# mttga/purejaxql

Measured on NVIDIA H100. Metric: MinAtar-Breakout env steps/sec @4096 envs x128 seeds, higher is better.
Workload: dtype f32

## Files before the change

purejaxql_b200/csrc/pqn_net.cu:

```cuda
#include <cuda_runtime.h>
#include <stdint.h>

#include "../../include/pqn_b200.h"
#include "api_common.h"
#include "tc_common.cuh"

namespace pqn {

constexpr int GT = 256;
constexpr int BK = 16;
constexpr float LN_EPS = 1e-6f;
constexpr int CONV_O = 16;
constexpr int CONV_PIX = 64;
constexpr int HID_CNN = 128;
constexpr int FLAT_CNN = CONV_PIX * CONV_O;

static int g_use_tc = 2;
static int g_conv_mma = 1;

__host__ __device__ static inline int64_t align4(int64_t x) { return (x + 3) & ~(int64_t)3; }

static int make_layout(const pqn_net_desc_t* d, pqn_net_layout_t* L) {
  int64_t off = 0;
  auto take = [&](int64_t n) { int64_t o = off; off += align4(n); return o; };
// ... 1050 lines not shown
      const uint32_t w0 = r00[(16 * i) * E::LD + ks], w1 = r00[(16 * i + 8) * E::LD + ks];
      a[i][0] = w0 & m_lo; a[i][1] = w1 & m_lo; a[i][2] = w0 & m_hi; a[i][3] = w1 & m_hi;
    }
    float2 bl[2], bh[2];
#pragma unroll
    for (int h = 0; h < 2; ++h) {
      bl[h] = wb_lo[(ks * 2 + h) * 32 + lane];
      bh[h] = wb_hi[(ks * 2 + h) * 32 + lane];
    }
#pragma unroll
    for (int h = 0; h < 2; ++h)
#pragma unroll
      for (int i = 0; i < 2; ++i) mma_tf32_16n8k8(z[i][h], a[i], __float_as_uint(bl[h].x), __float_as_uint(bl[h].y));
#pragma unroll
    for (int h = 0; h < 2; ++h)
#pragma unroll
      for (int i = 0; i < 2; ++i) mma_tf32_16n8k8(z[i][h], a[i], __float_as_uint(bh[h].x), __float_as_uint(bh[h].y));
  }
}

__device__ __forceinline__ void ln16_quad(const float (&z)[2][4], float& mean0, float& rstd0, float& mean1,
                                          float& rstd1) {
  float s0 = z[0][0] + z[0][1] + z[1][0] + z[1][1];
  float q0 = z[0][0] * z[0][0] + z[0][1] * z[0][1] + z[1][0] * z[1][0] + z[1][1] * z[1][1];
  float s1 = z[0][2] + z[0][3] + z[1][2] + z[1][3];
  float q1 = z[0][2] * z[0][2] + z[0][3] * z[0][3] + z[1][2] * z[1][2] + z[1][3] * z[1][3];
#pragma unroll
  for (int o = 1; o <= 2; o <<= 1) {
    s0 += __shfl_xor_sync(0xffffffffu, s0, o); q0 += __shfl_xor_sync(0xffffffffu, q0, o);
    s1 += __shfl_xor_sync(0xffffffffu, s1, o); q1 += __shfl_xor_sync(0xffffffffu, q1, o);
  }
  mean0 = s0 * (1.0f / CONV_O); mean1 = s1 * (1.0f / CONV_O);
  rstd0 = rsqrtf(fmaxf(q0 * (1.0f / CONV_O) - mean0 * mean0, 0.f) + LN_EPS);
  rstd1 = rsqrtf(fmaxf(q1 * (1.0f / CONV_O) - mean1 * mean1, 0.f) + LN_EPS);
}

constexpr int CONV_MMA_WARPS = 8;

template <int C, bool TRAIN, bool H16 = false>
__global__ void __launch_bounds__(CONV_MMA_WARPS * 32, 3)
    conv_fwd_mma_kernel(const uint32_t* __restrict__ obs, int64_t obs_rows_per_seed, const int32_t* __restrict__ gather,
                        const float* __restrict__ params, int64_t P, pqn_net_layout_t L, float* __restrict__ H1,
                        float* __restrict__ H1LO, float* __restrict__ XH1, float* __restrict__ RS1,
                        uint32_t* __restrict__ RB, float* __restrict__ bn_sums, int rows) {
  using Cfg = ConvCfg<C>;
  using M = ConvMma<C>;
  __shared__ float2 wb_hi[M::KS * 2 * 32], wb_lo[M::KS * 2 * 32];
  __shared__ float cb[CONV_O], sc[CONV_O], bi[CONV_O];
  __shared__ uint32_t so[CONV_MMA_WARPS][Cfg::SW];
  __shared__ uint32_t sxp[CONV_MMA_WARPS][CONV_PIX * ExpPatch<C>::LD];
  __shared__ float s_cnt[C];
  const int tid = threadIdx.x, warp = tid >> 5, lane = tid & 31;
  const int g = lane >> 2, t = lane & 3;
  const int seed = blockIdx.y;
  conv_mma_load_weights<C, true>(params + (int64_t)seed * P, L, wb_hi, wb_lo, cb, sc, bi);
  if (TRAIN && tid < C) s_cnt[tid] = 0.f;
  __syncthreads();
// ... 170 lines not shown
#pragma unroll
  for (int b = 0; b < 2 * Conv16<C>::KS; ++b) {
    const int o = 8 * b;
    uint32_t v = (o >> 5) < W ? w[(o >> 5) < W ? (o >> 5) : 0] : 0u;
    const int sh = o & 31;
    const uint32_t lo = sh >= 10 ? v >> (sh - 10) : v << (10 - sh);
    const uint32_t hi = sh + 4 <= 26 ? v << (26 - sh - 4) : v >> (sh + 4 - 26);
    out[b] = __byte_perm(lo, hi, 0x7610);
  }
}

template <int C>
__device__ __forceinline__ void store_patch16(const uint32_t* __restrict__ so, int pix, uint32_t* __restrict__ row) {
  using M = Conv16<C>;
  uint32_t w[M::ROW];
#pragma unroll
  for (int k = 0; k < M::ROW; ++k) w[k] = 0u;
  build_patch16<C>(so, pix, w);
#pragma unroll
  for (int q = 0; q < M::ROW / 4; ++q)
    *reinterpret_cast<uint4*>(row + 4 * q) = make_uint4(w[4 * q], w[4 * q + 1], w[4 * q + 2], w[4 * q + 3]);
}

template <int C>
__device__ __forceinline__ void conv16_block2(const uint32_t* __restrict__ xp, const uint4* __restrict__ wb,
                                              const float* __restrict__ cb, int mbp, int lane, float (&z)[2][2][4]) {
  using M = Conv16<C>;
  const int g = lane >> 2, t = lane & 3;
  const uint32_t mask = (1u << (10 + t)) | (1u << (26 + t));
#pragma unroll
  for (int i = 0; i < 2; ++i)
#pragma unroll
    for (int h = 0; h < 2; ++h) {
      z[i][h][0] = z[i][h][2] = cb[4 * t + 2 * h];
      z[i][h][1] = z[i][h][3] = cb[4 * t + 2 * h + 1];
    }
  const uint32_t* r00 = xp + (32 * mbp + g) * M::ROW;
#pragma unroll
  for (int s = 0; s < M::KS; ++s) {
    uint32_t a[2][4];
#pragma unroll
    for (int i = 0; i < 2; ++i) {
      const uint2 w0 = *reinterpret_cast<const uint2*>(r00 + (16 * i) * M::ROW + 2 * s);
      const uint2 w1 = *reinterpret_cast<const uint2*>(r00 + (16 * i + 8) * M::ROW + 2 * s);
      a[i][0] = w0.x & mask; a[i][1] = w1.x & mask; a[i][2] = w0.y & mask; a[i][3] = w1.y & mask;
    }
    uint4 b[2];
#pragma unroll
    for (int h = 0; h < 2; ++h) b[h] = wb[(s * 2 + h) * 32 + lane];
#pragma unroll
    for (int h = 0; h < 2; ++h)
#pragma unroll
      for (int i = 0; i < 2; ++i) mma_f16_16n8k16(z[i][h], a[i], b[h].z, b[h].w);
#pragma unroll
    for (int h = 0; h < 2; ++h)
#pragma unroll
      for (int i = 0; i < 2; ++i) mma_f16_16n8k16(z[i][h], a[i], b[h].x, b[h].y);
  }
}

__device__ __forceinline__ uint32_t cvt_f16x2_satfinite(float lo, float hi) {
  uint32_t r;
  asm("cvt.rn.satfinite.f16x2.f32 %0, %1, %2;" : "=r"(r) : "f"(hi), "f"(lo));
  return r;
}

constexpr int CONV16_WARPS = 4;
constexpr int CONV16_CTAS_PER_SM = 5;

template <int C, bool TRAIN, bool H16>
__global__ void __launch_bounds__(CONV16_WARPS * 32, CONV16_CTAS_PER_SM)
    conv_fwd_mma16_kernel(const uint32_t* __restrict__ obs, int64_t obs_rows_per_seed, const int32_t* __restrict__ gather,
                          const float* __restrict__ params, int64_t P, pqn_net_layout_t L, float* __restrict__ H1,
                          float* __restrict__ H1LO, float* __restrict__ XH1, float* __restrict__ RS1,
                          uint32_t* __restrict__ RB, float* __restrict__ bn_sums, int rows) {
  using Cfg = ConvCfg<C>;
  using M = Conv16<C>;
  __shared__ __align__(16) uint4 wb[M::KS * 2 * 32];
  __shared__ float cb[CONV_O], sc[CONV_O], bi[CONV_O];
  __shared__ uint32_t so[CONV16_WARPS][Cfg::SW];
  __shared__ __align__(16) uint32_t sxp[CONV16_WARPS][CONV_PIX * M::ROW];
  __shared__ float s_cnt[C];
  const int tid = threadIdx.x, warp = tid >> 5, lane = tid & 31;
  const int g = lane >> 2, t = lane & 3;
  const int seed = blockIdx.y;
  conv16_load_weights<C>(params + (int64_t)seed * P, L, wb, cb, sc, bi);
  if (TRAIN && tid < C) s_cnt[tid] = 0.f;
  __syncthreads();
  int cnt[C];
  uint32_t cmask[C];
#pragma unroll
  for (int c = 0; c < C; ++c) {
    cnt[c] = 0;
    cmask[c] = 0u;
    if (TRAIN) {
      for (int b = 0; b < 32; ++b) {
        const int f = lane * 32 + b;
        if (f < Cfg::OBS_BITS && f % C == c) cmask[c] |= 1u << b;
// ... 11 lines not shown
  auto fetch_obs = [&](int src) -> uint32_t {
    return __ldg(obs + ((int64_t)seed * obs_rows_per_seed + src) * Cfg::PW + (lane < Cfg::PW ? lane : 0));
  };
  const int row0 = blockIdx.x * CONV16_WARPS + warp;
  uint32_t pre = fetch_obs(fetch_index(row0));
  int src_next = fetch_index(row0 + row_stride);
  for (int row = row0; row < rows; row += row_stride) {
    __syncwarp();
    if (lane < Cfg::PW) my_so[lane] = pre;
    if (TRAIN && bn_sums != nullptr) {
#pragma unroll
      for (int c = 0; c < C; ++c) cnt[c] += __popc(pre & cmask[c]);
    }
    __syncwarp();
    pre = fetch_obs(src_next);
    src_next = fetch_index(row + 2 * row_stride);
    store_patch16<C>(my_so, lane, sxp[warp] + lane * M::ROW);
    store_patch16<C>(my_so, lane + 32, sxp[warp] + (lane + 32) * M::ROW);
    __syncwarp();
    const int64_t grow = (int64_t)seed * rows + row;
    float* __restrict__ hrow = H16 ? nullptr : H1 + grow * FLAT_CNN;
    __half* __restrict__ hrow16 = H16 ? reinterpret_cast<__half*>(H1) + grow * FLAT_CNN : nullptr;
    __half* __restrict__ lrow16 = H16 ? reinterpret_cast<__half*>(H1LO) + grow * FLAT_CNN : nullptr;
    float* __restrict__ xrow = (TRAIN && XH1) ? XH1 + grow * FLAT_CNN : nullptr;
    float* __restrict__ rrow = (TRAIN && RS1) ? RS1 + grow * CONV_PIX : nullptr;
    uint16_t* __restrict__ brow = (TRAIN && RB) ? reinterpret_cast<uint16_t*>(RB + grow * (FLAT_CNN / 32)) : nullptr;
    float keep_rs0 = 0.f, keep_rs1 = 0.f;
    uint32_t keep_rb = 0u;
#pragma unroll 1
    for (int mbp = 0; mbp < 2; ++mbp) {
      float z2[2][2][4];
      conv16_block2<C>(sxp[warp], wb, cb, mbp, lane, z2);
#pragma unroll
      for (int mi = 0; mi < 2; ++mi) {
        const int mb = 2 * mbp + mi;
        float (&z)[2][4] = z2[mi];
        float mean0, rstd0, mean1, rstd1;
        ln16_quad(z, mean0, rstd0, mean1, rstd1);
        const float nm0 = -mean0 * rstd0, nm1 = -mean1 * rstd1;
        uint32_t rb0 = 0u, rb1 = 0u;
        const int p0 = 16 * mb + g, p1 = p0 + 8, o4 = 4 * t;
        float x0[4], x1[4], v0[4], v1[4];
#pragma unroll
        for (int h = 0; h < 2; ++h) {
#pragma unroll
          for (int c = 0; c < 2; ++c) {
            const int o = o4 + 2 * h + c;
            x0[2 * h + c] = fmaf(z[h][c], rstd0, nm0);
            x1[2 * h + c] = fmaf(z[h][2 + c], rstd1, nm1);
            v0[2 * h + c] = fmaxf(fmaf(x0[2 * h + c], sc[o], bi[o]), 0.f);
            v1[2 * h + c] = fmaxf(fmaf(x1[2 * h + c], sc[o], bi[o]), 0.f);
          }
        }
        if (H16) {
          uint32_t hw0[2], hw1[2], lw0[2], lw1[2];
#pragma unroll
          for (int h = 0; h < 2; ++h) {
            hw0[h] = cvt_f16x2_satfinite(v0[2 * h], v0[2 * h + 1]);
            hw1[h] = cvt_f16x2_satfinite(v1[2 * h], v1[2 * h + 1]);
            const float2 f0 = __half22float2(*reinterpret_cast<const __half2*>(&hw0[h]));
            const float2 f1 = __half22float2(*reinterpret_cast<const __half2*>(&hw1[h]));
            const __half2 l0 = __floats2half2_rn((v0[2 * h] - f0.x) * tc::TC_LO_SCALE, (v0[2 * h + 1] - f0.y) * tc::TC_LO_SCALE);
            const __half2 l1 = __floats2half2_rn((v1[2 * h] - f1.x) * tc::TC_LO_SCALE, (v1[2 * h + 1] - f1.y) * tc::TC_LO_SCALE);
            lw0[h] = *reinterpret_cast<const uint32_t*>(&l0); lw1[h] = *reinterpret_cast<const uint32_t*>(&l1);
          }
          *reinterpret_cast<uint2*>(hrow16 + p0 * CONV_O + o4) = make_uint2(hw0[0], hw0[1]);
          *reinterpret_cast<uint2*>(lrow16 + p0 * CONV_O + o4) = make_uint2(lw0[0], lw0[1]);
          *reinterpret_cast<uint2*>(hrow16 + p1 * CONV_O + o4) = make_uint2(hw1[0], hw1[1]);
          *reinterpret_cast<uint2*>(lrow16 + p1 * CONV_O + o4) = make_uint2(lw1[0], lw1[1]);
        } else {
          *reinterpret_cast<float4*>(hrow + p0 * CONV_O + o4) = make_float4(v0[0], v0[1], v0[2], v0[3]);
          *reinterpret_cast<float4*>(hrow + p1 * CONV_O + o4) = make_float4(v1[0], v1[1], v1[2], v1[3]);
        }
        if (TRAIN) {
#pragma unroll
          for (int c = 0; c < 4; ++c) {
            rb0 |= (v0[c] > 0.f ? 1u : 0u) << (o4 + c);
            rb1 |= (v1[c] > 0.f ? 1u : 0u) << (o4 + c);
          }
        }
        if (xrow) {
          *reinterpret_cast<float4*>(xrow + p0 * CONV_O + o4) = make_float4(x0[0], x0[1], x0[2], x0[3]);
          *reinterpret_cast<float4*>(xrow + p1 * CONV_O + o4) = make_float4(x1[0], x1[1], x1[2], x1[3]);
          if (t == mb) { keep_rs0 = rstd0; keep_rs1 = rstd1; }
        }
        if (TRAIN && brow) {
          uint32_t rb = rb0 | (rb1 << 16);
          rb |= __shfl_xor_sync(0xffffffffu, rb, 1);
          rb |= __shfl_xor_sync(0xffffffffu, rb, 2);
          if (t == mb) keep_rb = rb;
        }
      }
    }
    if (TRAIN) {
      if (rrow) { rrow[16 * t + g] = keep_rs0; rrow[16 * t + g + 8] = keep_rs1; }
      if (brow) { brow[16 * t + g] = (uint16_t)keep_rb; brow[16 * t + g + 8] = (uint16_t)(keep_rb >> 16); }
    }
  }
  if (TRAIN && bn_sums != nullptr) {
#pragma unroll
    for (int c = 0; c < C; ++c) {
      int v = cnt[c];
#pragma unroll
      for (int o = 16; o > 0; o >>= 1) v += __shfl_xor_sync(0xffffffffu, v, o);
      if (lane == 0 && v) atomicAdd(&s_cnt[c], (float)v);
    }
    __syncthreads();
    if (tid < C && s_cnt[tid] != 0.f) {
      atomicAdd(bn_sums + (int64_t)seed * 2 * C + tid, s_cnt[tid]);
      atomicAdd(bn_sums + (int64_t)seed * 2 * C + C + tid, s_cnt[tid]);
    }
  }
}

constexpr int CDZ_LD = 16;
__device__ __forceinline__ int cswz(int p, int col) { return col ^ (((p >> 1) & 1) << 3); }

__device__ __forceinline__ void cp_async16(void* smem_dst, const void* gsrc) {
  asm volatile("cp.async.cg.shared.global [%0], [%1], 16;" ::"r"((uint32_t)__cvta_generic_to_shared(smem_dst)), "l"(gsrc)
               : "memory");
// ... 211 lines not shown
    if (warp == w && g == 0) {
#pragma unroll
      for (int col = 0; col < 4; ++col) {
        const int o = 8 * (col >> 1) + 2 * t + (col & 1);
        s_red[o] = (w == 0 ? 0.f : s_red[o]) + a_dsc[col];
        s_red[CONV_O + o] = (w == 0 ? 0.f : s_red[CONV_O + o]) + a_dbi[col];
        s_red[2 * CONV_O + o] = (w == 0 ? 0.f : s_red[2 * CONV_O + o]) + a_dcb[col];
      }
    }
    __syncthreads();
  }
  float* __restrict__ o = part + ((int64_t)seed * gridDim.x + blockIdx.x) * (M::TAPS * CONV_O + 3 * CONV_O);
  for (int i = tid; i < M::TAPS * CONV_O; i += blockDim.x) o[i] = s_w[i] * (1.0f / 255.0f);
  if (tid < 3 * CONV_O) o[M::TAPS * CONV_O + tid] = s_red[tid];
}

template <int C>
struct ConvBwd16 {
  static constexpr int MT = ConvMma<C>::MT;
  static constexpr int NG = 4 * MT;
  static constexpr int NGP = (NG % 8 == 4) ? NG : NG + 4;
  static constexpr int DY = 0;
  static constexpr int XH = DY + FLAT_CNN;
  static constexpr int RS = XH + FLAT_CNN;
  static constexpr int DZT = RS + CONV_PIX;
  static constexpr int PW = DZT + 2 * CONV_O * 32;
  static constexpr int WARP_FLOATS = (PW + 32 * NGP + 3) / 4 * 4;
  static constexpr int WARPS = (C == 4) ? 8 : 6;
  static constexpr int BYTES = (WARPS * WARP_FLOATS + 4 * CONV_O) * 4;
};

__device__ __forceinline__ int cswz16(int p, int col) {
  return ((p ^ ((p >> 2) & 1)) << 4) + (col ^ (((p >> 1) & 1) << 3));
}
__device__ __forceinline__ int dzt_word(int ch, int ks, int pos) {
  const int c7 = ch & 7;
  return (ch << 5) + ((ks ^ ((c7 + (c7 >> 2)) & 3)) << 3) + pos;
}

template <int C>
__global__ void __launch_bounds__(ConvBwd16<C>::WARPS * 32, 2)
    conv_bwd_mma16_kernel(const uint32_t* __restrict__ obs, int64_t obs_rows_per_seed, const int32_t* __restrict__ gather,
                          const float* __restrict__ params, int64_t P, pqn_net_layout_t L, const float* __restrict__ DY1,
                          const float* __restrict__ XH1, const float* __restrict__ RS1, float* __restrict__ part,
                          int rows, float gs) {
  using Cfg = ConvCfg<C>;
  using M = ConvMma<C>;
  using SM = ConvBwd16<C>;
  constexpr int PWD = PatchCfg<C>::WORDS;
  extern __shared__ __align__(16) float smem_bwd[];
  const int tid = threadIdx.x, warp = tid >> 5, lane = tid & 31;
  const int g = lane >> 2, t = lane & 3;
  const int seed = blockIdx.y;
  float* my = smem_bwd + warp * SM::WARP_FLOATS;
  float* my_dy = my + SM::DY;
  float* my_xh = my + SM::XH;
  float* my_rs = my + SM::RS;
  uint32_t* my_dzt = reinterpret_cast<uint32_t*>(my + SM::DZT);
  uint32_t* my_so = reinterpret_cast<uint32_t*>(my + SM::DZT);
  uint32_t* my_pw = reinterpret_cast<uint32_t*>(my + SM::PW);
  float* sc = smem_bwd + SM::WARPS * SM::WARP_FLOATS;
  float* s_red = sc + CONV_O;
  float* s_w = smem_bwd;
  static_assert(Cfg::SW <= 2 * CONV_O * 32, "obs staging aliases the dz planes");
  static_assert(M::MT * 16 * CONV_O <= SM::WARP_FLOATS * SM::WARPS, "dW reduction buffer aliases the warp slices");
  static_assert(Cfg::PW <= 32, "one packed observation word per lane");
  if (tid < CONV_O) sc[tid] = __ldg(params + (int64_t)seed * P + L.ln0_scale + tid);
  if (tid < 3 * CONV_O) s_red[tid] = 0.f;
  __syncthreads();
  float a_dsc[4] = {0.f, 0.f, 0.f, 0.f}, a_dbi[4] = {0.f, 0.f, 0.f, 0.f}, a_dcb[4] = {0.f, 0.f, 0.f, 0.f};
  float wrun[M::MT][2][4];
#pragma unroll
  for (int mt = 0; mt < M::MT; ++mt)
#pragma unroll
    for (int h = 0; h < 2; ++h)
#pragma unroll
      for (int j = 0; j < 4; ++j) wrun[mt][h][j] = 0.f;
  const uint32_t amask = (1u << (10 + (g & 3))) | (1u << (26 + (g & 3)));
  const int pos_g = g < 4 ? 2 * g : 2 * (g - 4) + 1;

  const int row_stride = gridDim.x * SM::WARPS;
  auto fetch_index = [&](int r) -> int {
    const int rc = r < rows ? r : rows - 1;
    return gather ? __ldg(gather + (int64_t)seed * rows + rc) : rc;
  };
  auto fetch_obs = [&](int src) -> uint32_t {
    return __ldg(obs + ((int64_t)seed * obs_rows_per_seed + src) * Cfg::PW + (lane < Cfg::PW ? lane : 0));
  };
  auto fetch_rows = [&](int r) {
    if (r < rows) {
      const int64_t gr = (int64_t)seed * rows + r;
      const float* dsrc = DY1 + gr * FLAT_CNN;
      const float* xsrc = XH1 + gr * FLAT_CNN;
#pragma unroll
      for (int i = 0; i < FLAT_CNN / 4 / 32; ++i) {
        const int q = i * 32 + lane, prow = q >> 2;
        const int dst = cswz16(prow, (q & 3) * 4);
        cp_async16(my_dy + dst, dsrc + q * 4);
        cp_async16(my_xh + dst, xsrc + q * 4);
      }
      if (lane < CONV_PIX / 4) cp_async16(my_rs + lane * 4, RS1 + gr * CONV_PIX + lane * 4);
    }
    cp_async_commit();
  };
  int row = blockIdx.x * SM::WARPS + warp;
  uint32_t pre = fetch_obs(fetch_index(row));
  int src_next = fetch_index(row + row_stride);
  fetch_rows(row);
  for (; row < rows; row += row_stride) {
    __syncwarp();
    if (lane < Cfg::PW) my_so[lane] = pre;
    if (lane == 0) my_so[Cfg::PW] = 0u;
    __syncwarp();
    pre = fetch_obs(src_next);
    src_next = fetch_index(row + 2 * row_stride);
    {
      uint32_t w0[PWD], w1[PWD];
      patch_bits<C>(my_so, 2 * lane, w0);
      patch_bits<C>(my_so, 2 * lane + 1, w1);
      uint32_t pw[SM::NGP];
#pragma unroll
      for (int k = 0; k < SM::NGP; ++k) pw[k] = 0u;
#pragma unroll
      for (int q = 0; q < SM::NG; ++q) {
        const int ql = q & 3, slot = (q & ~3) + (ql == 1 ? 2 : (ql == 2 ? 1 : ql));
        const int bit = 4 * q, wi = bit >> 5, sh = bit & 31;
        if (wi < PWD) {
          const uint32_t v0 = w0[wi < PWD ? wi : 0], v1 = w1[wi < PWD ? wi : 0];
          const uint32_t lo = sh >= 10 ? v0 >> (sh >= 10 ? sh - 10 : 0) : v0 << (sh < 10 ? 10 - sh : 0);
          const uint32_t hi = sh <= 26 ? v1 << (sh <= 26 ? 26 - sh : 0) : v1 >> (sh > 26 ? sh - 26 : 0);
          pw[slot] = __byte_perm(lo, hi, 0x7610);
        }
      }
      uint32_t* dstw = my_pw + lane * SM::NGP;
#pragma unroll
      for (int k = 0; k < SM::NGP / 4; ++k)
        *reinterpret_cast<uint4*>(dstw + 4 * k) = make_uint4(pw[4 * k], pw[4 * k + 1], pw[4 * k + 2], pw[4 * k + 3]);
    }
    cp_async_wait_all();
    __syncwarp();
#pragma unroll 1
    for (int mb = 0; mb < 4; ++mb) {
      const int p0 = 16 * mb + 2 * g, p1 = p0 + 1;
      float z[2][4];
      float2 dyv[2][2];
#pragma unroll
      for (int h = 0; h < 2; ++h) {
        dyv[h][0] = *reinterpret_cast<const float2*>(my_dy + cswz16(p0, 8 * h + 2 * t));
        dyv[h][1] = *reinterpret_cast<const float2*>(my_dy + cswz16(p1, 8 * h + 2 * t));
        const float2 a0 = *reinterpret_cast<const float2*>(my_xh + cswz16(p0, 8 * h + 2 * t));
        const float2 a1 = *reinterpret_cast<const float2*>(my_xh + cswz16(p1, 8 * h + 2 * t));
        z[h][0] = a0.x; z[h][1] = a0.y; z[h][2] = a1.x; z[h][3] = a1.y;
      }
      const float rstd0 = my_rs[p0] * gs, rstd1 = my_rs[p1] * gs;
      float dxh[2][4];
      float m1a = 0.f, m2a = 0.f, m1b = 0.f, m2b = 0.f;
#pragma unroll
      for (int h = 0; h < 2; ++h) {
        const int o = 8 * h + 2 * t;
        const float dy4[4] = {dyv[h][0].x, dyv[h][0].y, dyv[h][1].x, dyv[h][1].y};
#pragma unroll
        for (int j = 0; j < 4; ++j) {
          const int col = 2 * h + (j & 1);
          a_dsc[col] = fmaf(dy4[j], z[h][j], a_dsc[col]);
          a_dbi[col] += dy4[j];
          dxh[h][j] = dy4[j] * sc[o + (j & 1)];
          if (j < 2) { m1a += dxh[h][j]; m2a = fmaf(dxh[h][j], z[h][j], m2a); }
          else { m1b += dxh[h][j]; m2b = fmaf(dxh[h][j], z[h][j], m2b); }
        }
      }
#pragma unroll
      for (int o = 1; o <= 2; o <<= 1) {
        m1a += __shfl_xor_sync(0xffffffffu, m1a, o); m2a += __shfl_xor_sync(0xffffffffu, m2a, o);
        m1b += __shfl_xor_sync(0xffffffffu, m1b, o); m2b += __shfl_xor_sync(0xffffffffu, m2b, o);
      }
      m1a *= (1.0f / CONV_O); m2a *= (1.0f / CONV_O); m1b *= (1.0f / CONV_O); m2b *= (1.0f / CONV_O);
#pragma unroll
      for (int h = 0; h < 2; ++h) {
        float dzv[4];
#pragma unroll
        for (int j = 0; j < 4; ++j) {
          const float rstd = j < 2 ? rstd0 : rstd1, m1 = j < 2 ? m1a : m1b, m2 = j < 2 ? m2a : m2b;
          dzv[j] = rstd * (dxh[h][j] - m1 - z[h][j] * m2);
          a_dcb[2 * h + (j & 1)] += dzv[j];
        }
#pragma unroll
        for (int c = 0; c < 2; ++c) {
          const float v0 = dzv[c], v1 = dzv[2 + c];
          const uint32_t hw = cvt_f16x2_satfinite(v0, v1);
          const float2 hf = __half22float2(*reinterpret_cast<const __half2*>(&hw));
          const __half2 lw = __floats2half2_rn(v0 - hf.x, v1 - hf.y);
          const int wd = dzt_word(8 * h + 2 * t + c, mb, pos_g);
          my_dzt[wd] = hw;
          my_dzt[CONV_O * 32 + wd] = *reinterpret_cast<const uint32_t*>(&lw);
        }
      }
    }
    __syncwarp();
    fetch_rows(row + row_stride);
    float wacc[M::MT][2][4];
#pragma unroll
    for (int mt = 0; mt < M::MT; ++mt)
#pragma unroll
      for (int h = 0; h < 2; ++h)
#pragma unroll
        for (int j = 0; j < 4; ++j) wacc[mt][h][j] = 0.f;
#pragma unroll 1
    for (int ks = 0; ks < 4; ++ks) {
      uint2 bhi[2], blo[2];
#pragma unroll
      for (int h = 0; h < 2; ++h) {
        const int wd = dzt_word(8 * h + g, ks, 2 * t);
        bhi[h] = *reinterpret_cast<const uint2*>(my_dzt + wd);
        blo[h] = *reinterpret_cast<const uint2*>(my_dzt + CONV_O * 32 + wd);
      }
      const uint32_t* pa = my_pw + (8 * ks + t) * SM::NGP + 2 * (g >> 2);
      const uint32_t* pb = pa + 4 * SM::NGP;
#pragma unroll
      for (int mt = 0; mt < M::MT; ++mt) {
        const uint2 wa = *reinterpret_cast<const uint2*>(pa + 4 * mt), wb = *reinterpret_cast<const uint2*>(pb + 4 * mt);
        uint32_t a[4];
        a[0] = wa.x & amask; a[1] = wa.y & amask; a[2] = wb.x & amask; a[3] = wb.y & amask;
// ... 289 lines not shown
}


template <int C>
static int launch_conv_bwd_mma(dim3 grid, cudaStream_t st, const uint32_t* obs, int64_t orps, const int32_t* gather,
                               const float* params, int64_t P, const pqn_net_layout_t& L, const float* dy1,
                               const float* xh1, const float* rs1, float* grads, float* part, int rows) {
  auto kfn = conv_bwd_mma_kernel<C>;
  if (cudaFuncSetAttribute(kfn, cudaFuncAttributeMaxDynamicSharedMemorySize, ConvBwdSmem<C>::BYTES) != cudaSuccess)
    return check_launch("conv_bwd_mma(cudaFuncSetAttribute)");
  kfn<<<grid, ConvBwdSmem<C>::WARPS * 32, ConvBwdSmem<C>::BYTES, st>>>(obs, orps, gather, params, P, L, dy1, xh1, rs1,
                                                                       part, rows);
  const int n = 9 * C * CONV_O + 3 * CONV_O;
  if (final_slices((int)grid.x) == 32)
    conv_bwd_final_kernel<32><<<dim3(cdiv(n, 8), grid.y), 256, 0, st>>>(part, (int)grid.x, 9 * C * CONV_O, grads, P, L);
  else
    conv_bwd_final_kernel<8><<<dim3(cdiv(n, 32), grid.y), 256, 0, st>>>(part, (int)grid.x, 9 * C * CONV_O, grads, P, L);
  return 0;
}

template <int C>
static int launch_conv_bwd_mma16(dim3 grid, cudaStream_t st, const uint32_t* obs, int64_t orps, const int32_t* gather,
                                 const float* params, int64_t P, const pqn_net_layout_t& L, const float* dy1,
                                 const float* xh1, const float* rs1, float* grads, float* part, int rows, float gs) {
  auto kfn = conv_bwd_mma16_kernel<C>;
  if (cudaFuncSetAttribute(kfn, cudaFuncAttributeMaxDynamicSharedMemorySize, ConvBwd16<C>::BYTES) != cudaSuccess)
    return check_launch("conv_bwd_mma16(cudaFuncSetAttribute)");
  kfn<<<grid, ConvBwd16<C>::WARPS * 32, ConvBwd16<C>::BYTES, st>>>(obs, orps, gather, params, P, L, dy1, xh1, rs1, part,
                                                                   rows, gs);
  const int n = 9 * C * CONV_O + 3 * CONV_O;
  if (final_slices((int)grid.x) == 32)
    conv_bwd_final_kernel<32><<<dim3(cdiv(n, 8), grid.y), 256, 0, st>>>(part, (int)grid.x, 9 * C * CONV_O, grads, P, L);
  else
    conv_bwd_final_kernel<8><<<dim3(cdiv(n, 32), grid.y), 256, 0, st>>>(part, (int)grid.x, 9 * C * CONV_O, grads, P, L);
  return 0;
}

static size_t row_bwd_smem(int N, int A, bool head) {
  return (size_t)(24 * N + (head ? A * N + 8 * A + 16 + 8 * A * N : 0)) * sizeof(float);
}
static int64_t row_bwd_part_floats(int N, int A) { return 3 * (int64_t)N + (int64_t)A * N + A + 2; }

template <int N, bool HEAD, typename... Args>
static int launch_row_bwd(dim3 grid, int A, cudaStream_t st, Args... args) {
  const size_t sm = row_bwd_smem(N, A, HEAD);
  if (sm > 48 * 1024 &&
      cudaFuncSetAttribute(row_bwd_kernel<N, HEAD>, cudaFuncAttributeMaxDynamicSharedMemorySize, (int)sm) != cudaSuccess)
    return check_launch("row_bwd(cudaFuncSetAttribute)");
  LaunchScope _ls(K_ROW_BWD, st);
  row_bwd_kernel<N, HEAD><<<grid, 256, sm, st>>>(args...);
  return 0;
}
// ... 41 lines not shown
  const int maxc = (rows + CONV_MMA_WARPS - 1) / CONV_MMA_WARPS;
  int best = 1;
  double best_eff = 0.0;
  const int lim = (6 * resident + S - 1) / S;
  for (int per_seed = 1; per_seed <= lim && per_seed <= maxc; ++per_seed) {
    const int total = per_seed * S;
    const int waves = (total + resident - 1) / resident;
    if (waves > 6) break;
    const double eff = (double)total / ((double)waves * resident);
    if (eff > best_eff + 0.01 || (eff > best_eff - 0.01 && waves <= 4)) { best_eff = eff > best_eff ? eff : best_eff; best = per_seed; }
  }
  return (unsigned)best;
}

template <bool TRAIN>
static int launch_conv_fwd(int C, dim3 grid, cudaStream_t st, const uint32_t* obs, int64_t orps, const int32_t* gather,
                           const float* params, int64_t P, const pqn_net_layout_t& L, float* h1, float* h1lo, float* bn,
                           int rows, float* xh1 = nullptr, float* rs1 = nullptr, uint32_t* rb = nullptr,
                           bool h16 = false) {
  if (g_conv_mma == 1) {
    const dim3 mg(conv_mma_ctas((int)grid.y, rows, CONV16_CTAS_PER_SM), grid.y);
    LaunchScope _ls(TRAIN ? K_CONV_FWD : K_CONV_FWD_INFER, st);
#define PQN_CONV16(CC)                                                                                              \
  if (h16) conv_fwd_mma16_kernel<CC, TRAIN, true><<<mg, CONV16_WARPS * 32, 0, st>>>(obs, orps, gather, params, P, L, h1, h1lo, xh1, rs1, rb, bn, rows); \
  else conv_fwd_mma16_kernel<CC, TRAIN, false><<<mg, CONV16_WARPS * 32, 0, st>>>(obs, orps, gather, params, P, L, h1, h1lo, xh1, rs1, rb, bn, rows)
    switch (C) {
      case 4: PQN_CONV16(4); break;
      case 6: PQN_CONV16(6); break;
      case 7: PQN_CONV16(7); break;
      case 10: PQN_CONV16(10); break;
      default: return -1;
    }
#undef PQN_CONV16
    return 0;
  }
  if (g_conv_mma == 3) {
    const dim3 mg(conv_mma_ctas((int)grid.y, rows, 3), grid.y);
    LaunchScope _ls(TRAIN ? K_CONV_FWD : K_CONV_FWD_INFER, st);
    switch (C) {
      case 4: conv_fwd_mma_kernel<4, TRAIN><<<mg, CONV_MMA_WARPS * 32, 0, st>>>(obs, orps, gather, params, P, L, h1, h1lo, xh1, rs1, rb, bn, rows); break;
      case 6: conv_fwd_mma_kernel<6, TRAIN><<<mg, CONV_MMA_WARPS * 32, 0, st>>>(obs, orps, gather, params, P, L, h1, h1lo, xh1, rs1, rb, bn, rows); break;
      case 7: conv_fwd_mma_kernel<7, TRAIN><<<mg, CONV_MMA_WARPS * 32, 0, st>>>(obs, orps, gather, params, P, L, h1, h1lo, xh1, rs1, rb, bn, rows); break;
      case 10: conv_fwd_mma_kernel<10, TRAIN><<<mg, CONV_MMA_WARPS * 32, 0, st>>>(obs, orps, gather, params, P, L, h1, h1lo, xh1, rs1, rb, bn, rows); break;
      default: return -1;
    }
    return 0;
  }
  switch (C) {
// ... 628 lines not shown
  const int64_t P = L.total;
  Workspace w;
  carve(d, S, rows, (char*)workspace, &w);
  const int A = d->num_actions;
  const int R = (int)rows;
  if (cudaMemsetAsync(grads, 0, (size_t)S * P * sizeof(float), st) != cudaSuccess)
    return check_launch("pqn_qnet_loss_grad(memset)");
  if (modular_net(d)) {
    nrm::NormWs nw;
    nrm::carve_norm(d, S, rows, (char*)workspace, &nw);
    return nrm::norm_loss_grad(d, L, params, batch_stats, obs, gather, obs_rows_per_seed, action, target, tr_rows_per_seed,
                              grads, loss_sum, qsa_sum, bn_sums, S, R, nw, st);
  }

  if (d->kind == PQN_NET_MINATAR_CNN) {
    const uint32_t* ob = (const uint32_t*)obs;
    const bool use_tc = g_use_tc && A <= PQN_TC_MAX_A;
    const bool f16 = use_tc && g_use_tc == 2;
    const Planes16 pl = planes16(w, S, rows);
    const bool conv16 = f16 && g_conv_mma == 1;
    const float gscale = f16 ? grad_scale(rows) : 1.0f;
    launch_conv_fwd<true>(d->in_c, dim3(cdiv(rows, 4), S), st, ob, obs_rows_per_seed, gather, params, P, L,
                          conv16 ? (float*)pl.h1_hi : w.h1, conv16 ? (float*)pl.h1_lo : nullptr, bn_sums, R,
                          g_conv_mma ? w.cxhat : nullptr, g_conv_mma ? w.crstd : nullptr,
                          (g_conv_mma == 1 || g_conv_mma == 3) ? w.relu_bits : nullptr, conv16);
    if (f16) {
      if (!conv16) launch_split16_h1(w.h1, pl, (int64_t)S * rows * FLAT_CNN, st);
      launch_split16_w1(params, P, L.d0_w, pl, S, st);
      if ((rc = tc16_dense_fwd(tc::EPI_LN_TRAIN, params, P, L, w, pl, A, nullptr, S, R, st))) return rc;
    } else if (use_tc) {
      launch_split_w1(params, P, L.d0_w, w.w1_lo, S, st);
      if ((rc = tc_dense_fwd(tc::EPI_LN_TRAIN, params, P, L, w, A, nullptr, S, R, st))) return rc;
    } else {
      if ((rc = launch_dense<1>(128, dim3(cdiv(rows, 128), S), st, w.h1, rows * FLAT_CNN, FLAT_CNN, params, P, L.d0_w, L.d0_b,
                      L.ln1_scale, L.ln1_bias, 0, 0, A, w.h2, w.xhat2, w.rstd2, nullptr, R, FLAT_CNN))) return rc;
    }
    const dim3 rbg(conv_mma_ctas(S, R, 4), S);
    if ((rc = run_row_bwd(128, true, rbg, A, st, w.h2, w.xhat2, w.rstd2, nullptr, w.dz2, (use_tc && !f16) ? w.dz2_lo : nullptr,
                          f16 ? pl.dz_hi : nullptr, f16 ? pl.dz_lo : nullptr, gscale, params, grads, P, L.ln1_scale,
                          L.ln1_bias, L.d0_b, L.head_w, L.head_b, gather, action, target, tr_rows_per_seed, loss_sum,
                          qsa_sum, w.rb_part, R))) return rc;
    if (f16) {
      if ((rc = tc16_wgrad(grads, P, L, pl, S, R, gscale, w.wg_part, st))) return rc;
      if ((rc = tc16_dgrad(w, pl, S, R, g_conv_mma == 1 || g_conv_mma == 3, gscale, st))) return rc;
    } else if (use_tc) {
      if ((rc = tc_wgrad(grads, P, L, w, S, R, st))) return rc;
      if ((rc = tc_dgrad(params, P, L, w, S, R, g_conv_mma == 1 || g_conv_mma == 3, st))) return rc;
    } else {
      const int splits = wgrad_splits(FLAT_CNN / 128, S, R);
      run_wgrad_ffma(w.h1, rows * FLAT_CNN, FLAT_CNN, w.dz2, rows * HID_CNN, HID_CNN, grads, P, L.d0_w, R, FLAT_CNN, S, splits, w.wg_part, st);
      launch_dgrad(w.dz2, rows * HID_CNN, HID_CNN, params, P, L.d0_w, w.h1, w.h1, rows * FLAT_CNN, R, FLAT_CNN, 0, S, st);
    }
    dim3 cg(conv_bwd_ctas(S, R), S);
    if (g_conv_mma) {
      const dim3 mg(conv_mma_ctas(S, R, 2), S);
      LaunchScope _ls(K_CONV_BWD, st);
      const float gs16 = grad_scale((int)rows) * (1.0f / 16.0f);
      if (g_conv_mma == 1) {
        switch (d->in_c) {
          case 4: rc = launch_conv_bwd_mma16<4>(mg, st, ob, obs_rows_per_seed, gather, params, P, L, w.h1, w.cxhat, w.crstd, grads, w.cb_part, R, gs16); break;
          case 6: rc = launch_conv_bwd_mma16<6>(mg, st, ob, obs_rows_per_seed, gather, params, P, L, w.h1, w.cxhat, w.crstd, grads, w.cb_part, R, gs16); break;
          case 7: rc = launch_conv_bwd_mma16<7>(mg, st, ob, obs_rows_per_seed, gather, params, P, L, w.h1, w.cxhat, w.crstd, grads, w.cb_part, R, gs16); break;
          case 10: rc = launch_conv_bwd_mma16<10>(mg, st, ob, obs_rows_per_seed, gather, params, P, L, w.h1, w.cxhat, w.crstd, grads, w.cb_part, R, gs16); break;
        }
      } else
      switch (d->in_c) {
        case 4: rc = launch_conv_bwd_mma<4>(mg, st, ob, obs_rows_per_seed, gather, params, P, L, w.h1, w.cxhat, w.crstd, grads, w.cb_part, R); break;
        case 6: rc = launch_conv_bwd_mma<6>(mg, st, ob, obs_rows_per_seed, gather, params, P, L, w.h1, w.cxhat, w.crstd, grads, w.cb_part, R); break;
        case 7: rc = launch_conv_bwd_mma<7>(mg, st, ob, obs_rows_per_seed, gather, params, P, L, w.h1, w.cxhat, w.crstd, grads, w.cb_part, R); break;
        case 10: rc = launch_conv_bwd_mma<10>(mg, st, ob, obs_rows_per_seed, gather, params, P, L, w.h1, w.cxhat, w.crstd, grads, w.cb_part, R); break;
      }
      if (rc) return rc;
    } else
    switch (d->in_c) {
      case 4: { LaunchScope _ls(K_CONV_BWD, st); conv_bwd_kernel<4><<<cg, 256, 0, st>>>(ob, obs_rows_per_seed, gather, params, P, L, w.h1, grads, R); } break;
      case 6: { LaunchScope _ls(K_CONV_BWD, st); conv_bwd_kernel<6><<<cg, 256, 0, st>>>(ob, obs_rows_per_seed, gather, params, P, L, w.h1, grads, R); } break;
      case 7: { LaunchScope _ls(K_CONV_BWD, st); conv_bwd_kernel<7><<<cg, 256, 0, st>>>(ob, obs_rows_per_seed, gather, params, P, L, w.h1, grads, R); } break;
      case 10: { LaunchScope _ls(K_CONV_BWD, st); conv_bwd_kernel<10><<<cg, 256, 0, st>>>(ob, obs_rows_per_seed, gather, params, P, L, w.h1, grads, R); } break;
    }
  } else {
    const int D = d->in_c, H = d->hidden;
    const int BM = (H == 128) ? 128 : 64;
    const bool bits = d->kind == PQN_NET_MLP_BITS, bits_tc = bits && g_use_tc == 2;
    const uint32_t* ob = (const uint32_t*)obs;
    bits::BitsWs bw = {};
    if (bits) bits::carve_bits(d, S, rows, (char*)workspace + carve(d, S, rows, nullptr, nullptr), &bw);
// ... 66 lines not shown
```

Before: 33.51 million.

## Recompute conv LayerNorm xhat and rstd in backward instead of storing them

```diff
diff --git a/purejaxql_b200/csrc/pqn_net.cu b/purejaxql_b200/csrc/pqn_net.cu
--- a/purejaxql_b200/csrc/pqn_net.cu
+++ b/purejaxql_b200/csrc/pqn_net.cu
@@ -1096,17 +1096,17 @@
 __device__ __forceinline__ void ln16_quad(const float (&z)[2][4], float& mean0, float& rstd0, float& mean1,
                                           float& rstd1) {
   float s0 = z[0][0] + z[0][1] + z[1][0] + z[1][1];
-  float q0 = z[0][0] * z[0][0] + z[0][1] * z[0][1] + z[1][0] * z[1][0] + z[1][1] * z[1][1];
+  float q0 = fmaf(z[1][1], z[1][1], fmaf(z[1][0], z[1][0], fmaf(z[0][0], z[0][0], __fmul_rn(z[0][1], z[0][1]))));
   float s1 = z[0][2] + z[0][3] + z[1][2] + z[1][3];
-  float q1 = z[0][2] * z[0][2] + z[0][3] * z[0][3] + z[1][2] * z[1][2] + z[1][3] * z[1][3];
+  float q1 = fmaf(z[1][3], z[1][3], fmaf(z[1][2], z[1][2], fmaf(z[0][2], z[0][2], __fmul_rn(z[0][3], z[0][3]))));
 #pragma unroll
   for (int o = 1; o <= 2; o <<= 1) {
     s0 += __shfl_xor_sync(0xffffffffu, s0, o); q0 += __shfl_xor_sync(0xffffffffu, q0, o);
     s1 += __shfl_xor_sync(0xffffffffu, s1, o); q1 += __shfl_xor_sync(0xffffffffu, q1, o);
   }
-  mean0 = s0 * (1.0f / CONV_O); mean1 = s1 * (1.0f / CONV_O);
-  rstd0 = rsqrtf(fmaxf(q0 * (1.0f / CONV_O) - mean0 * mean0, 0.f) + LN_EPS);
-  rstd1 = rsqrtf(fmaxf(q1 * (1.0f / CONV_O) - mean1 * mean1, 0.f) + LN_EPS);
+  mean0 = __fmul_rn(s0, 1.0f / CONV_O); mean1 = __fmul_rn(s1, 1.0f / CONV_O);
+  rstd0 = rsqrtf(fmaxf(fmaf(q0, 1.0f / CONV_O, -__fmul_rn(mean0, mean0)), 0.f) + LN_EPS);
+  rstd1 = rsqrtf(fmaxf(fmaf(q1, 1.0f / CONV_O, -__fmul_rn(mean1, mean1)), 0.f) + LN_EPS);
 }
 
 constexpr int CONV_MMA_WARPS = 8;
@@ -1323,25 +1323,25 @@
     *reinterpret_cast<uint4*>(row + 4 * q) = make_uint4(w[4 * q], w[4 * q + 1], w[4 * q + 2], w[4 * q + 3]);
 }
 
-template <int C>
-__device__ __forceinline__ void conv16_block2(const uint32_t* __restrict__ xp, const uint4* __restrict__ wb,
-                                              const float* __restrict__ cb, int mbp, int lane, float (&z)[2][2][4]) {
+template <int C, int NB>
+__device__ __forceinline__ void conv16_blocks(const uint32_t* __restrict__ xp, const uint4* __restrict__ wb,
+                                              const float* __restrict__ cb, int mb0, int lane, float (&z)[NB][2][4]) {
   using M = Conv16<C>;
   const int g = lane >> 2, t = lane & 3;
   const uint32_t mask = (1u << (10 + t)) | (1u << (26 + t));
 #pragma unroll
-  for (int i = 0; i < 2; ++i)
+  for (int i = 0; i < NB; ++i)
 #pragma unroll
     for (int h = 0; h < 2; ++h) {
       z[i][h][0] = z[i][h][2] = cb[4 * t + 2 * h];
       z[i][h][1] = z[i][h][3] = cb[4 * t + 2 * h + 1];
     }
-  const uint32_t* r00 = xp + (32 * mbp + g) * M::ROW;
+  const uint32_t* r00 = xp + (16 * mb0 + g) * M::ROW;
 #pragma unroll
   for (int s = 0; s < M::KS; ++s) {
-    uint32_t a[2][4];
-#pragma unroll
-    for (int i = 0; i < 2; ++i) {
+    uint32_t a[NB][4];
+#pragma unroll
+    for (int i = 0; i < NB; ++i) {
       const uint2 w0 = *reinterpret_cast<const uint2*>(r00 + (16 * i) * M::ROW + 2 * s);
       const uint2 w1 = *reinterpret_cast<const uint2*>(r00 + (16 * i + 8) * M::ROW + 2 * s);
       a[i][0] = w0.x & mask; a[i][1] = w1.x & mask; a[i][2] = w0.y & mask; a[i][3] = w1.y & mask;
@@ -1352,12 +1352,26 @@
 #pragma unroll
     for (int h = 0; h < 2; ++h)
 #pragma unroll
-      for (int i = 0; i < 2; ++i) mma_f16_16n8k16(z[i][h], a[i], b[h].z, b[h].w);
+      for (int i = 0; i < NB; ++i) mma_f16_16n8k16(z[i][h], a[i], b[h].z, b[h].w);
 #pragma unroll
     for (int h = 0; h < 2; ++h)
 #pragma unroll
-      for (int i = 0; i < 2; ++i) mma_f16_16n8k16(z[i][h], a[i], b[h].x, b[h].y);
-  }
+      for (int i = 0; i < NB; ++i) mma_f16_16n8k16(z[i][h], a[i], b[h].x, b[h].y);
+  }
+}
+
+__device__ __forceinline__ void conv16_xhat(const float (&z)[2][4], float (&x0)[4], float (&x1)[4], float& rstd0,
+                                            float& rstd1) {
+  float mean0, mean1;
+  ln16_quad(z, mean0, rstd0, mean1, rstd1);
+  const float nm0 = -__fmul_rn(mean0, rstd0), nm1 = -__fmul_rn(mean1, rstd1);
+#pragma unroll
+  for (int h = 0; h < 2; ++h)
+#pragma unroll
+    for (int c = 0; c < 2; ++c) {
+      x0[2 * h + c] = fmaf(z[h][c], rstd0, nm0);
+      x1[2 * h + c] = fmaf(z[h][2 + c], rstd1, nm1);
+    }
 }
 
 __device__ __forceinline__ uint32_t cvt_f16x2_satfinite(float lo, float hi) {
@@ -1373,8 +1387,7 @@
 __global__ void __launch_bounds__(CONV16_WARPS * 32, CONV16_CTAS_PER_SM)
     conv_fwd_mma16_kernel(const uint32_t* __restrict__ obs, int64_t obs_rows_per_seed, const int32_t* __restrict__ gather,
                           const float* __restrict__ params, int64_t P, pqn_net_layout_t L, float* __restrict__ H1,
-                          float* __restrict__ H1LO, float* __restrict__ XH1, float* __restrict__ RS1,
-                          uint32_t* __restrict__ RB, float* __restrict__ bn_sums, int rows) {
+                          float* __restrict__ H1LO, uint32_t* __restrict__ RB, float* __restrict__ bn_sums, int rows) {
   using Cfg = ConvCfg<C>;
   using M = Conv16<C>;
   __shared__ __align__(16) uint4 wb[M::KS * 2 * 32];
@@ -1432,35 +1445,24 @@
     float* __restrict__ hrow = H16 ? nullptr : H1 + grow * FLAT_CNN;
     __half* __restrict__ hrow16 = H16 ? reinterpret_cast<__half*>(H1) + grow * FLAT_CNN : nullptr;
     __half* __restrict__ lrow16 = H16 ? reinterpret_cast<__half*>(H1LO) + grow * FLAT_CNN : nullptr;
-    float* __restrict__ xrow = (TRAIN && XH1) ? XH1 + grow * FLAT_CNN : nullptr;
-    float* __restrict__ rrow = (TRAIN && RS1) ? RS1 + grow * CONV_PIX : nullptr;
     uint16_t* __restrict__ brow = (TRAIN && RB) ? reinterpret_cast<uint16_t*>(RB + grow * (FLAT_CNN / 32)) : nullptr;
-    float keep_rs0 = 0.f, keep_rs1 = 0.f;
     uint32_t keep_rb = 0u;
 #pragma unroll 1
     for (int mbp = 0; mbp < 2; ++mbp) {
       float z2[2][2][4];
-      conv16_block2<C>(sxp[warp], wb, cb, mbp, lane, z2);
+      conv16_blocks<C, 2>(sxp[warp], wb, cb, 2 * mbp, lane, z2);
 #pragma unroll
       for (int mi = 0; mi < 2; ++mi) {
         const int mb = 2 * mbp + mi;
-        float (&z)[2][4] = z2[mi];
-        float mean0, rstd0, mean1, rstd1;
-        ln16_quad(z, mean0, rstd0, mean1, rstd1);
-        const float nm0 = -mean0 * rstd0, nm1 = -mean1 * rstd1;
+        float x0[4], x1[4], rstd0, rstd1;
+        conv16_xhat(z2[mi], x0, x1, rstd0, rstd1);
         uint32_t rb0 = 0u, rb1 = 0u;
         const int p0 = 16 * mb + g, p1 = p0 + 8, o4 = 4 * t;
-        float x0[4], x1[4], v0[4], v1[4];
-#pragma unroll
-        for (int h = 0; h < 2; ++h) {
-#pragma unroll
-          for (int c = 0; c < 2; ++c) {
-            const int o = o4 + 2 * h + c;
-            x0[2 * h + c] = fmaf(z[h][c], rstd0, nm0);
-            x1[2 * h + c] = fmaf(z[h][2 + c], rstd1, nm1);
-            v0[2 * h + c] = fmaxf(fmaf(x0[2 * h + c], sc[o], bi[o]), 0.f);
-            v1[2 * h + c] = fmaxf(fmaf(x1[2 * h + c], sc[o], bi[o]), 0.f);
-          }
+        float v0[4], v1[4];
+#pragma unroll
+        for (int c = 0; c < 4; ++c) {
+          v0[c] = fmaxf(fmaf(x0[c], sc[o4 + c], bi[o4 + c]), 0.f);
+          v1[c] = fmaxf(fmaf(x1[c], sc[o4 + c], bi[o4 + c]), 0.f);
         }
         if (H16) {
           uint32_t hw0[2], hw1[2], lw0[2], lw1[2];
@@ -1489,11 +1491,6 @@
             rb1 |= (v1[c] > 0.f ? 1u : 0u) << (o4 + c);
           }
         }
-        if (xrow) {
-          *reinterpret_cast<float4*>(xrow + p0 * CONV_O + o4) = make_float4(x0[0], x0[1], x0[2], x0[3]);
-          *reinterpret_cast<float4*>(xrow + p1 * CONV_O + o4) = make_float4(x1[0], x1[1], x1[2], x1[3]);
-          if (t == mb) { keep_rs0 = rstd0; keep_rs1 = rstd1; }
-        }
         if (TRAIN && brow) {
           uint32_t rb = rb0 | (rb1 << 16);
           rb |= __shfl_xor_sync(0xffffffffu, rb, 1);
@@ -1502,10 +1499,7 @@
         }
       }
     }
-    if (TRAIN) {
-      if (rrow) { rrow[16 * t + g] = keep_rs0; rrow[16 * t + g + 8] = keep_rs1; }
-      if (brow) { brow[16 * t + g] = (uint16_t)keep_rb; brow[16 * t + g + 8] = (uint16_t)(keep_rb >> 16); }
-    }
+    if (TRAIN && brow) { brow[16 * t + g] = (uint16_t)keep_rb; brow[16 * t + g + 8] = (uint16_t)(keep_rb >> 16); }
   }
   if (TRAIN && bn_sums != nullptr) {
 #pragma unroll
@@ -1763,12 +1757,14 @@
   static constexpr int NGP = (NG % 8 == 4) ? NG : NG + 4;
   static constexpr int DY = 0;
   static constexpr int XH = DY + FLAT_CNN;
-  static constexpr int RS = XH + FLAT_CNN;
-  static constexpr int DZT = RS + CONV_PIX;
+  static constexpr int RS = XH + 16 * CONV_O;
+  static constexpr int DZT = RS + 16;
   static constexpr int PW = DZT + 2 * CONV_O * 32;
-  static constexpr int WARP_FLOATS = (PW + 32 * NGP + 3) / 4 * 4;
+  static constexpr int XP = PW + 32 * NGP;
+  static constexpr int WARP_FLOATS = (XP + CONV_PIX * Conv16<C>::ROW + 3) / 4 * 4;
   static constexpr int WARPS = (C == 4) ? 8 : 6;
-  static constexpr int BYTES = (WARPS * WARP_FLOATS + 4 * CONV_O) * 4;
+  static constexpr int WB = WARPS * WARP_FLOATS;
+  static constexpr int BYTES = (WB + Conv16<C>::KS * 2 * 32 * 4 + 6 * CONV_O) * 4;
 };
 
 __device__ __forceinline__ int cswz16(int p, int col) {
@@ -1783,8 +1779,7 @@
 __global__ void __launch_bounds__(ConvBwd16<C>::WARPS * 32, 2)
     conv_bwd_mma16_kernel(const uint32_t* __restrict__ obs, int64_t obs_rows_per_seed, const int32_t* __restrict__ gather,
                           const float* __restrict__ params, int64_t P, pqn_net_layout_t L, const float* __restrict__ DY1,
-                          const float* __restrict__ XH1, const float* __restrict__ RS1, float* __restrict__ part,
-                          int rows, float gs) {
+                          float* __restrict__ part, int rows, float gs) {
   using Cfg = ConvCfg<C>;
   using M = ConvMma<C>;
   using SM = ConvBwd16<C>;
@@ -1800,13 +1795,18 @@
   uint32_t* my_dzt = reinterpret_cast<uint32_t*>(my + SM::DZT);
   uint32_t* my_so = reinterpret_cast<uint32_t*>(my + SM::DZT);
   uint32_t* my_pw = reinterpret_cast<uint32_t*>(my + SM::PW);
-  float* sc = smem_bwd + SM::WARPS * SM::WARP_FLOATS;
-  float* s_red = sc + CONV_O;
+  uint32_t* my_xp = reinterpret_cast<uint32_t*>(my + SM::XP);
+  uint4* wb = reinterpret_cast<uint4*>(smem_bwd + SM::WB);
+  float* cb = smem_bwd + SM::WB + Conv16<C>::KS * 2 * 32 * 4;
+  float* sc = cb + CONV_O;
+  float* bi = sc + CONV_O;
+  float* s_red = bi + CONV_O;
   float* s_w = smem_bwd;
   static_assert(Cfg::SW <= 2 * CONV_O * 32, "obs staging aliases the dz planes");
   static_assert(M::MT * 16 * CONV_O <= SM::WARP_FLOATS * SM::WARPS, "dW reduction buffer aliases the warp slices");
   static_assert(Cfg::PW <= 32, "one packed observation word per lane");
-  if (tid < CONV_O) sc[tid] = __ldg(params + (int64_t)seed * P + L.ln0_scale + tid);
+  static_assert(SM::XP % 4 == 0 && SM::WB % 4 == 0, "16-byte aligned patch rows and weight fragments");
+  conv16_load_weights<C>(params + (int64_t)seed * P, L, wb, cb, sc, bi);
   if (tid < 3 * CONV_O) s_red[tid] = 0.f;
   __syncthreads();
   float a_dsc[4] = {0.f, 0.f, 0.f, 0.f}, a_dbi[4] = {0.f, 0.f, 0.f, 0.f}, a_dcb[4] = {0.f, 0.f, 0.f, 0.f};
@@ -1828,26 +1828,21 @@
   auto fetch_obs = [&](int src) -> uint32_t {
     return __ldg(obs + ((int64_t)seed * obs_rows_per_seed + src) * Cfg::PW + (lane < Cfg::PW ? lane : 0));
   };
-  auto fetch_rows = [&](int r) {
+  auto fetch_dy = [&](int r) {
     if (r < rows) {
-      const int64_t gr = (int64_t)seed * rows + r;
-      const float* dsrc = DY1 + gr * FLAT_CNN;
-      const float* xsrc = XH1 + gr * FLAT_CNN;
+      const float* dsrc = DY1 + ((int64_t)seed * rows + r) * FLAT_CNN;
 #pragma unroll
       for (int i = 0; i < FLAT_CNN / 4 / 32; ++i) {
         const int q = i * 32 + lane, prow = q >> 2;
-        const int dst = cswz16(prow, (q & 3) * 4);
-        cp_async16(my_dy + dst, dsrc + q * 4);
-        cp_async16(my_xh + dst, xsrc + q * 4);
-      }
-      if (lane < CONV_PIX / 4) cp_async16(my_rs + lane * 4, RS1 + gr * CONV_PIX + lane * 4);
+        cp_async16(my_dy + cswz16(prow, (q & 3) * 4), dsrc + q * 4);
+      }
     }
     cp_async_commit();
   };
   int row = blockIdx.x * SM::WARPS + warp;
   uint32_t pre = fetch_obs(fetch_index(row));
   int src_next = fetch_index(row + row_stride);
-  fetch_rows(row);
+  fetch_dy(row);
   for (; row < rows; row += row_stride) {
     __syncwarp();
     if (lane < Cfg::PW) my_so[lane] = pre;
@@ -1855,6 +1850,8 @@
     __syncwarp();
     pre = fetch_obs(src_next);
     src_next = fetch_index(row + 2 * row_stride);
+    store_patch16<C>(my_so, lane, my_xp + lane * Conv16<C>::ROW);
+    store_patch16<C>(my_so, lane + 32, my_xp + (lane + 32) * Conv16<C>::ROW);
     {
       uint32_t w0[PWD], w1[PWD];
       patch_bits<C>(my_so, 2 * lane, w0);
@@ -1882,6 +1879,16 @@
     __syncwarp();
 #pragma unroll 1
     for (int mb = 0; mb < 4; ++mb) {
+      {
+        float zc[1][2][4], x0[4], x1[4], rs0, rs1;
+        conv16_blocks<C, 1>(my_xp, wb, cb, mb, lane, zc);
+        conv16_xhat(zc[0], x0, x1, rs0, rs1);
+        __syncwarp();
+        *reinterpret_cast<float4*>(my_xh + cswz16(g, 4 * t)) = make_float4(x0[0], x0[1], x0[2], x0[3]);
+        *reinterpret_cast<float4*>(my_xh + cswz16(g + 8, 4 * t)) = make_float4(x1[0], x1[1], x1[2], x1[3]);
+        if (t == 0) { my_rs[g] = rs0; my_rs[g + 8] = rs1; }
+        __syncwarp();
+      }
       const int p0 = 16 * mb + 2 * g, p1 = p0 + 1;
       float z[2][4];
       float2 dyv[2][2];
@@ -1889,11 +1896,11 @@
       for (int h = 0; h < 2; ++h) {
         dyv[h][0] = *reinterpret_cast<const float2*>(my_dy + cswz16(p0, 8 * h + 2 * t));
         dyv[h][1] = *reinterpret_cast<const float2*>(my_dy + cswz16(p1, 8 * h + 2 * t));
-        const float2 a0 = *reinterpret_cast<const float2*>(my_xh + cswz16(p0, 8 * h + 2 * t));
-        const float2 a1 = *reinterpret_cast<const float2*>(my_xh + cswz16(p1, 8 * h + 2 * t));
+        const float2 a0 = *reinterpret_cast<const float2*>(my_xh + cswz16(2 * g, 8 * h + 2 * t));
+        const float2 a1 = *reinterpret_cast<const float2*>(my_xh + cswz16(2 * g + 1, 8 * h + 2 * t));
         z[h][0] = a0.x; z[h][1] = a0.y; z[h][2] = a1.x; z[h][3] = a1.y;
       }
-      const float rstd0 = my_rs[p0] * gs, rstd1 = my_rs[p1] * gs;
+      const float rstd0 = my_rs[2 * g] * gs, rstd1 = my_rs[2 * g + 1] * gs;
       float dxh[2][4];
       float m1a = 0.f, m2a = 0.f, m1b = 0.f, m2b = 0.f;
 #pragma unroll
@@ -1938,7 +1945,7 @@
       }
     }
     __syncwarp();
-    fetch_rows(row + row_stride);
+    fetch_dy(row + row_stride);
     float wacc[M::MT][2][4];
 #pragma unroll
     for (int mt = 0; mt < M::MT; ++mt)
@@ -2274,12 +2281,11 @@
 template <int C>
 static int launch_conv_bwd_mma16(dim3 grid, cudaStream_t st, const uint32_t* obs, int64_t orps, const int32_t* gather,
                                  const float* params, int64_t P, const pqn_net_layout_t& L, const float* dy1,
-                                 const float* xh1, const float* rs1, float* grads, float* part, int rows, float gs) {
+                                 float* grads, float* part, int rows, float gs) {
   auto kfn = conv_bwd_mma16_kernel<C>;
   if (cudaFuncSetAttribute(kfn, cudaFuncAttributeMaxDynamicSharedMemorySize, ConvBwd16<C>::BYTES) != cudaSuccess)
     return check_launch("conv_bwd_mma16(cudaFuncSetAttribute)");
-  kfn<<<grid, ConvBwd16<C>::WARPS * 32, ConvBwd16<C>::BYTES, st>>>(obs, orps, gather, params, P, L, dy1, xh1, rs1, part,
-                                                                   rows, gs);
+  kfn<<<grid, ConvBwd16<C>::WARPS * 32, ConvBwd16<C>::BYTES, st>>>(obs, orps, gather, params, P, L, dy1, part, rows, gs);
   const int n = 9 * C * CONV_O + 3 * CONV_O;
   if (final_slices((int)grid.x) == 32)
     conv_bwd_final_kernel<32><<<dim3(cdiv(n, 8), grid.y), 256, 0, st>>>(part, (int)grid.x, 9 * C * CONV_O, grads, P, L);
@@ -2367,8 +2373,8 @@
     const dim3 mg(conv_mma_ctas((int)grid.y, rows, CONV16_CTAS_PER_SM), grid.y);
     LaunchScope _ls(TRAIN ? K_CONV_FWD : K_CONV_FWD_INFER, st);
 #define PQN_CONV16(CC)                                                                                              \
-  if (h16) conv_fwd_mma16_kernel<CC, TRAIN, true><<<mg, CONV16_WARPS * 32, 0, st>>>(obs, orps, gather, params, P, L, h1, h1lo, xh1, rs1, rb, bn, rows); \
-  else conv_fwd_mma16_kernel<CC, TRAIN, false><<<mg, CONV16_WARPS * 32, 0, st>>>(obs, orps, gather, params, P, L, h1, h1lo, xh1, rs1, rb, bn, rows)
+  if (h16) conv_fwd_mma16_kernel<CC, TRAIN, true><<<mg, CONV16_WARPS * 32, 0, st>>>(obs, orps, gather, params, P, L, h1, h1lo, rb, bn, rows); \
+  else conv_fwd_mma16_kernel<CC, TRAIN, false><<<mg, CONV16_WARPS * 32, 0, st>>>(obs, orps, gather, params, P, L, h1, h1lo, rb, bn, rows)
     switch (C) {
       case 4: PQN_CONV16(4); break;
       case 6: PQN_CONV16(6); break;
@@ -3043,7 +3049,7 @@
     const float gscale = f16 ? grad_scale(rows) : 1.0f;
     launch_conv_fwd<true>(d->in_c, dim3(cdiv(rows, 4), S), st, ob, obs_rows_per_seed, gather, params, P, L,
                           conv16 ? (float*)pl.h1_hi : w.h1, conv16 ? (float*)pl.h1_lo : nullptr, bn_sums, R,
-                          g_conv_mma ? w.cxhat : nullptr, g_conv_mma ? w.crstd : nullptr,
+                          g_conv_mma == 3 ? w.cxhat : nullptr, g_conv_mma == 3 ? w.crstd : nullptr,
                           (g_conv_mma == 1 || g_conv_mma == 3) ? w.relu_bits : nullptr, conv16);
     if (f16) {
       if (!conv16) launch_split16_h1(w.h1, pl, (int64_t)S * rows * FLAT_CNN, st);
@@ -3079,10 +3085,10 @@
       const float gs16 = grad_scale((int)rows) * (1.0f / 16.0f);
       if (g_conv_mma == 1) {
         switch (d->in_c) {
-          case 4: rc = launch_conv_bwd_mma16<4>(mg, st, ob, obs_rows_per_seed, gather, params, P, L, w.h1, w.cxhat, w.crstd, grads, w.cb_part, R, gs16); break;
-          case 6: rc = launch_conv_bwd_mma16<6>(mg, st, ob, obs_rows_per_seed, gather, params, P, L, w.h1, w.cxhat, w.crstd, grads, w.cb_part, R, gs16); break;
-          case 7: rc = launch_conv_bwd_mma16<7>(mg, st, ob, obs_rows_per_seed, gather, params, P, L, w.h1, w.cxhat, w.crstd, grads, w.cb_part, R, gs16); break;
-          case 10: rc = launch_conv_bwd_mma16<10>(mg, st, ob, obs_rows_per_seed, gather, params, P, L, w.h1, w.cxhat, w.crstd, grads, w.cb_part, R, gs16); break;
+          case 4: rc = launch_conv_bwd_mma16<4>(mg, st, ob, obs_rows_per_seed, gather, params, P, L, w.h1, grads, w.cb_part, R, gs16); break;
+          case 6: rc = launch_conv_bwd_mma16<6>(mg, st, ob, obs_rows_per_seed, gather, params, P, L, w.h1, grads, w.cb_part, R, gs16); break;
+          case 7: rc = launch_conv_bwd_mma16<7>(mg, st, ob, obs_rows_per_seed, gather, params, P, L, w.h1, grads, w.cb_part, R, gs16); break;
+          case 10: rc = launch_conv_bwd_mma16<10>(mg, st, ob, obs_rows_per_seed, gather, params, P, L, w.h1, grads, w.cb_part, R, gs16); break;
         }
       } else
       switch (d->in_c) {
```

Result: faster. 35.55 million, median of 6 (+6.1%).
